# 2361098148/LocoManipulationRL

Hardware: AMD Instinct MI355X
Metric: env-steps/sec (whole node), horizontal-locomotion 4096 envs (higher is better)
Workload: dtype f32

## Files before the change

locomanipulationrl_amd/csrc/lm_dynamics.h:

```cpp
#pragma once
#include "lm_samplers.h"

#if defined(LM_STAMPS) && LM_STAMPS != 2
#define LM_STAMP(k) do { __builtin_amdgcn_sched_barrier(0); unsigned long long t_; \
    asm volatile("s_memtime %0\n\ts_waitcnt lgkmcnt(0)" : "=s"(t_) :: "memory"); __builtin_amdgcn_sched_barrier(0); \
    if (threadIdx.x == 0) { lm_stamp_lds[k] += t_ - lm_stamp_lds[15]; lm_stamp_lds[15] = t_; } } while (0)
#else
#define LM_STAMP(k) do { } while (0)
#endif

#define HUB_FLOATS 10
#define ENVS_PER_WAVE 16
#define PUB_LIMB_STRIDE 123
#define LIMB_STRIDE 124
#define T_J0 0
#define T_P1 14
#define T_P2 40
#define T_I0 66
#define T_Q1 76
#define T_Q2 96
#define T_TIP 116
#define T_FOOT 119
#define T_FLAG 122
#define LM_ITAB_FLOATS (HUB_FLOATS + 4 * LIMB_STRIDE)
// ... 243 lines not shown
    Wf[0] = Wl[0] + b0; Wf[1] = Wl[1] + a0.x; Wf[2] = Wl[2] + a0.y;
    Wf[3] = Wl[3] + a1.x; Wf[4] = Wl[4] + a1.y; Wf[5] = Wl[5] + a2.y;
  }
  const float imu = mu > 0.f ? 1.0f / mu : 0.f;
  const float nrW0 = -1.0f / Wf[0]; G.W0t = mk2(Wf[1], Wf[2]); G.nrWt = mk2(-imu / Wf[3], -imu / Wf[5]);
  pgs_cross_blocks<0>(limb, T, X, Wf, G.X0[0], G.X12[0]); pgs_cross_blocks<1>(limb, T, X, Wf, G.X0[1], G.X12[1]);
  pgs_cross_blocks<2>(limb, T, X, Wf, G.X0[2], G.X12[2]); pgs_cross_blocks<3>(limb, T, X, Wf, G.X0[3], G.X12[3]);
#pragma unroll
  for (int k = 0; k < 4; k++) { G.X0[k][0] *= nrW0; G.X0[k][1] *= mu * nrW0; G.X0[k][2] *= mu * nrW0; G.X12[k][1] = sp2(mu) * G.X12[k][1]; G.X12[k][2] = sp2(mu) * G.X12[k][2]; }
  S.lam0 = 0.f; S.lam12 = sp2(0.f);
  S.c0 = (vf[0] + bn) * nrW0; S.c12 = mk2(vf[1], vf[2]);
  S.m0 = limb == 0 ? 1.f : 0.f; S.m1 = limb == 1 ? 1.f : 0.f; S.m2 = limb == 2 ? 1.f : 0.f; S.m3 = limb == 3 ? 1.f : 0.f;
}
LM_DEV void pgs_sweeps(PgsState& S, int it0, int it1) {
  for (int it = it0; it < it1; it += 2) {
    pgs_turn<0>(S.m0, S.G, S.lam0, S.lam12, S.c0, S.c12);
    pgs_turn<1>(S.m1, S.G, S.lam0, S.lam12, S.c0, S.c12);
    pgs_turn<2>(S.m2, S.G, S.lam0, S.lam12, S.c0, S.c12);
    pgs_turn<3>(S.m3, S.G, S.lam0, S.lam12, S.c0, S.c12);
    if (it + 1 < it1) {
      pgs_turn<3>(S.m3, S.G, S.lam0, S.lam12, S.c0, S.c12);
      pgs_turn<2>(S.m2, S.G, S.lam0, S.lam12, S.c0, S.c12);
      pgs_turn<1>(S.m1, S.G, S.lam0, S.lam12, S.c0, S.c12);
      pgs_turn<0>(S.m0, S.G, S.lam0, S.lam12, S.c0, S.c12);
    }
  }
}
LM_DEV void pgs_finish(const PgsState& S, float mu, const R4 X[6], float lam[3], float w[6]) {
  const f2 l12 = sp2(mu) * S.lam12;
  lam[0] = S.lam0; lam[1] = l12.x; lam[2] = l12.y;
#pragma unroll
  for (int i = 0; i < 6; i++) { const f2 t = l12 * X[i].q; w[i] = quad_sum(fmaf(S.lam0, X[i].p.y, t.x + t.y)); }
}

struct FreeBody { V3 p; Q4 q; SV u; };

LM_DEV void integrate_free(FreeBody& F, const M3& R, float dt) {
  V3 ww = mul(R, F.u.w);
  float wn = sqrtf(dot(ww, ww)), th = wn * dt;
  Q4 dq;
  if (th < 1e-8f) { dq.w = 1.f; dq.x = 0.5f * dt * ww.x; dq.y = 0.5f * dt * ww.y; dq.z = 0.5f * dt * ww.z; }
  else { float sh, ch; lm_sincos(0.5f * th, &sh, &ch); float s = sh / wn; dq.w = ch; dq.x = s * ww.x; dq.y = s * ww.y; dq.z = s * ww.z; }
  Q4 qn = qmul(dq, F.q);
  float rn = rsqrtf(qn.w * qn.w + qn.x * qn.x + qn.y * qn.y + qn.z * qn.z);
  F.q.w = qn.w * rn; F.q.x = qn.x * rn; F.q.y = qn.y * rn; F.q.z = qn.z * rn;
  M3 Rn = quat_to_mat(F.q.w, F.q.x, F.q.y, F.q.z);
  F.p = fma3(dt, mul(Rn, F.u.v), F.p);
}

#ifdef LM_WAVES2
#define STASH_SLOTS 18
#define LM_STEP_ATTR __attribute__((amdgpu_waves_per_eu(2, 2)))
#elif defined(LM_HELPER_WAVE)
#define STASH_SLOTS 29
#define HAND_IN 22
#define HAND_OUT 26
#define LM_STEP_ATTR
#else
#define STASH_SLOTS 22
#define LM_STEP_ATTR
#endif
struct Stash {
  float4* base; int lane;
  LM_DEV void put(int slot, float a, float b, float c, float d) const { base[slot * 64 + lane] = make_float4(a, b, c, d); }
  LM_DEV float4 get(int slot) const { return base[slot * 64 + lane]; }
};
#ifdef LM_HELPER_WAVE
LM_DEV void hw_barrier() {
  __builtin_amdgcn_sched_barrier(0);
  asm volatile("" ::: "memory");
  __builtin_amdgcn_s_waitcnt(0xc07f);
  __builtin_amdgcn_s_barrier();
  asm volatile("" ::: "memory");
  __builtin_amdgcn_sched_barrier(0);
}
#endif
LM_DEV void stash_sv3(const Stash& S, int slot, SV a, SV b, SV c, float e0 = 0.f, float e1 = 0.f) {
  S.put(slot + 0, a.w.x, a.w.y, a.w.z, a.v.x); S.put(slot + 1, a.v.y, a.v.z, b.w.x, b.w.y);
  S.put(slot + 2, b.w.z, b.v.x, b.v.y, b.v.z); S.put(slot + 3, c.w.x, c.w.y, c.w.z, c.v.x); S.put(slot + 4, c.v.y, c.v.z, e0, e1);
}
LM_DEV void unstash_sv3(const Stash& S, int slot, SV& a, SV& b, SV& c) {
  float4 t0 = S.get(slot), t1 = S.get(slot + 1), t2 = S.get(slot + 2), t3 = S.get(slot + 3), t4 = S.get(slot + 4);
  a = sv(v3(t0.x, t0.y, t0.z), v3(t0.w, t1.x, t1.y)); b = sv(v3(t1.z, t1.w, t2.x), v3(t2.y, t2.z, t2.w)); c = sv(v3(t3.x, t3.y, t3.z), v3(t3.w, t4.x, t4.y));
}

#if defined(LM_PASS0_STASH) || defined(LM_WAVES2)
#define LM_PASS0_REG 0
#else
#define LM_PASS0_REG 1
#endif
struct PassTerms {
  S6 Fq0, Fq1, Fq2;
  float Ha[6], hq[3];
  float Jq0[3]; f2 j12[3];
  R4 PB[6];
  SI Isc;
};
LM_DEV S6 s6(SV a) { S6 r; r.a = mk2(a.w.x, a.w.y); r.b = mk2(a.w.z, a.v.x); r.c = mk2(a.v.y, a.v.z); return r; }
#define LM_PASS_ROWS(I, b, r0, r1, r2) { \
  I.PB[0].p = mk2(b.w.x, r0.w.x); I.PB[1].p = mk2(b.w.y, r0.w.y); I.PB[2].p = mk2(b.w.z, r0.w.z); \
  I.PB[3].p = mk2(b.v.x, r0.v.x); I.PB[4].p = mk2(b.v.y, r0.v.y); I.PB[5].p = mk2(b.v.z, r0.v.z); \
  I.PB[0].q = mk2(r1.w.x, r2.w.x); I.PB[1].q = mk2(r1.w.y, r2.w.y); I.PB[2].q = mk2(r1.w.z, r2.w.z); \
  I.PB[3].q = mk2(r1.v.x, r2.v.x); I.PB[4].q = mk2(r1.v.y, r2.v.y); I.PB[5].q = mk2(r1.v.z, r2.v.z); }
LM_DEV void pin(float& x) { asm("" : "+v"(x)); }
LM_DEV void pin(f2& x) { asm("" : "+v"(x)); }
LM_DEV void pin(S6& x) { pin(x.a); pin(x.b); pin(x.c); }
template <int MODE> LM_DEV void pin_terms(PassTerms& I) {
  pin(I.Fq0); pin(I.Fq1); pin(I.Fq2);
  pin(I.Ha[0]); pin(I.Ha[1]); pin(I.Ha[2]); pin(I.Ha[3]); pin(I.Ha[4]); pin(I.Ha[5]);
  pin(I.hq[0]); pin(I.hq[1]); pin(I.hq[2]); pin(I.Jq0[0]); pin(I.Jq0[1]); pin(I.Jq0[2]); pin(I.j12[0]); pin(I.j12[1]); pin(I.j12[2]);
  pin(I.PB[0].p); pin(I.PB[1].p); pin(I.PB[2].p); pin(I.PB[3].p); pin(I.PB[4].p); pin(I.PB[5].p);
  pin(I.PB[0].q); pin(I.PB[1].q); pin(I.PB[2].q); pin(I.PB[3].q); pin(I.PB[4].q); pin(I.PB[5].q);
  if (MODE == 0) { pin(I.Isc.m); pin(I.Isc.h.x); pin(I.Isc.h.y); pin(I.Isc.h.z); pin(I.Isc.xx); pin(I.Isc.yy); pin(I.Isc.zz); pin(I.Isc.xy); pin(I.Isc.xz); pin(I.Isc.yz); }
// ... 29 lines not shown
  St.put(4, I.Fq2.c.x, I.Fq2.c.y, 0.f, 0.f);
  St.put(5, I.Ha[0], I.Ha[1], I.Ha[2], I.Ha[3]); St.put(6, I.Ha[4], I.Ha[5], 0.f, 0.f);
  St.put(16, I.Isc.m, I.Isc.h.x, I.Isc.h.y, I.Isc.h.z); St.put(17, I.Isc.xx, I.Isc.yy, I.Isc.zz, I.Isc.xy); St.put(18, I.Isc.xz, I.Isc.yz, 0.f, 0.f);
}
#endif
template <int MODE> LM_DEV void unstash_terms(const Stash& St, PassTerms& I) {
  asm volatile("" ::: "memory");
  float isc_xz = 0.f, isc_yz = 0.f;
  {
    const float4 t0 = St.get(0), t1 = St.get(1), t2 = St.get(2), t3 = St.get(3), t4 = St.get(4);
    isc_xz = t4.z; isc_yz = t4.w;
    I.Fq0.a = mk2(t0.x, t0.y); I.Fq0.b = mk2(t0.z, t0.w); I.Fq0.c = mk2(t1.x, t1.y);
    I.Fq1.a = mk2(t1.z, t1.w); I.Fq1.b = mk2(t2.x, t2.y); I.Fq1.c = mk2(t2.z, t2.w);
    I.Fq2.a = mk2(t3.x, t3.y); I.Fq2.b = mk2(t3.z, t3.w); I.Fq2.c = mk2(t4.x, t4.y);
  }
  const float4 h5 = St.get(5), h6 = St.get(6), h7 = St.get(7), h8 = St.get(8), h9 = St.get(9);
  I.Ha[0] = h5.x; I.Ha[1] = h5.y; I.Ha[2] = h5.z; I.Ha[3] = h5.w; I.Ha[4] = h6.x; I.Ha[5] = h6.y;
  I.hq[0] = h6.z; I.hq[1] = h6.w; I.hq[2] = h7.x;
  I.Jq0[0] = h7.y; I.Jq0[1] = h7.z; I.Jq0[2] = h7.w;
  I.j12[0] = mk2(h8.x, h8.y); I.j12[1] = mk2(h8.z, h8.w); I.j12[2] = mk2(h9.x, h9.y);
  {
    const float4 g0 = St.get(10), g1 = St.get(11), g2 = St.get(12), g3 = St.get(13), g4 = St.get(14), g5 = St.get(15);
    I.PB[0].p = mk2(g0.x, g0.y); I.PB[1].p = mk2(g0.z, g0.w); I.PB[2].p = mk2(g1.x, g1.y); I.PB[3].p = mk2(g1.z, g1.w); I.PB[4].p = mk2(g2.x, g2.y); I.PB[5].p = mk2(g2.z, g2.w);
    I.PB[0].q = mk2(g3.x, g3.y); I.PB[1].q = mk2(g3.z, g3.w); I.PB[2].q = mk2(g4.x, g4.y); I.PB[3].q = mk2(g4.z, g4.w); I.PB[4].q = mk2(g5.x, g5.y); I.PB[5].q = mk2(g5.z, g5.w);
  }
  if (MODE == 0) {
#ifdef LM_WAVES2
    const float4 g16 = St.get(16), g17 = St.get(17), g18 = make_float4(isc_xz, isc_yz, 0.f, 0.f);
#else
    const float4 g16 = St.get(16), g17 = St.get(17), g18 = St.get(18); (void)isc_xz; (void)isc_yz;
#endif
    I.Isc.m = g16.x; I.Isc.h = v3(g16.y, g16.z, g16.w); I.Isc.xx = g17.x; I.Isc.yy = g17.y; I.Isc.zz = g17.z; I.Isc.xy = g17.w; I.Isc.xz = g18.x; I.Isc.yz = g18.y;
  }
}

template <class T> struct PlateInvT { V3T<T> ii, c; T im; };
LM_DEV PlateInvT<float> plate_inv(const lm_params* __restrict__ P, float m, float s) {
  PlateInvT<float> Q; Q.ii = v3(1.0f / (s * P->plate_inertia[0]), 1.0f / (s * P->plate_inertia[1]), 1.0f / (s * P->plate_inertia[2]));
  Q.c = v3(P->plate_com[0], P->plate_com[1], P->plate_com[2]); Q.im = 1.0f / m; return Q;
}
template <class T> LM_DEV void plate_inv_apply(const PlateInvT<T>& Q, V3T<T> n, V3T<T> f, V3T<T>& al, V3T<T>& a) {
  const V3T<T> nc = n - cross(Q.c, f);
  al = v3t<T>(nc.x * Q.ii.x, nc.y * Q.ii.y, nc.z * Q.ii.z);
  a = fma3(Q.im, f, cross(Q.c, al));
}
LM_DEV SI plate_inertia_env(const lm_params* __restrict__ P, float m, float s) {
  const V3 c = v3(P->plate_com[0], P->plate_com[1], P->plate_com[2]); const float cc = dot(c, c);
  SI I; I.m = m; I.h = m * c;
  I.xx = fmaf(m, cc - c.x * c.x, s * P->plate_inertia[0]); I.yy = fmaf(m, cc - c.y * c.y, s * P->plate_inertia[1]); I.zz = fmaf(m, cc - c.z * c.z, s * P->plate_inertia[2]);
  I.xy = -m * c.x * c.y; I.xz = -m * c.x * c.z; I.yz = -m * c.y * c.z;
  return I;
}

template <int MODE, int VAR, int DR, int CF, int HW = 0>
LM_DEV void substep_pass(const lm_params* __restrict__ P, int limb, const FreeBody& F, const PassTerms& I, float dt, float kd, const float cjv[3],
                         const bool sat[3], const float tsat[3], const float tgt[3], const float qd[3], float bn, float mu_dr,
                         bool mp_on, float m_plate, float s_plate, float qdn[3], SV& un, float lamc[3], const Stash* Hd = nullptr) {
  const S6 Fq0 = I.Fq0, Fq1 = I.Fq1, Fq2 = I.Fq2;
  float Ha[6] = {I.Ha[0], I.Ha[1], I.Ha[2], I.Ha[3], I.Ha[4], I.Ha[5]}, r[3];
  const float hq[3] = {I.hq[0], I.hq[1], I.hq[2]};
  R4 PBh[6];
  const float Jq_[3][3] = {{I.Jq0[0], I.Jq0[1], I.Jq0[2]}, {I.j12[0].x, I.j12[1].x, I.j12[2].x}, {I.j12[0].y, I.j12[1].y, I.j12[2].y}};
  const f2 j12_[3] = {I.j12[0], I.j12[1], I.j12[2]};
  float Jqh[3][3]; f2 j12h[3]; float bnh = bn;
  const float (*Jq)[3] = HW == 2 ? Jqh : Jq_;
  const f2* j12 = HW == 2 ? j12h : j12_;
  const R4* PB = HW ? PBh : I.PB;
  const int di[3] = {0, 3, 5};
#pragma unroll
  for (int a = 0; a < 3; a++) {
    const float cj = cjv[a];
    {
#pragma clang fp contract(off)
      Ha[di[a]] = fmaf(dt, sat[a] ? cj : kd + cj, Ha[di[a]]);
      const float rr = sat[a] ? tsat[a] : kd * (tgt[a] - qd[a]);
      const float damp = cj * qd[a];
      r[a] = HW ? rr - damp : (rr - damp) - hq[a];
    }
  }
  float Hi[6]; inv3sym(Ha, Hi);
  const S6 K0 = fma6(Hi[0], Fq0, fma6(Hi[1], Fq1, Hi[2] * Fq2));
  const S6 K1 = fma6(Hi[1], Fq0, fma6(Hi[3], Fq1, Hi[4] * Fq2));
  const S6 K2 = fma6(Hi[2], Fq0, fma6(Hi[4], Fq1, Hi[5] * Fq2));
  float qdd[3], qdf[3], v0f[6], vf[3];
  R4 T[6], X[6];
  if (MODE == 0) {
    float A0[6][6]; si_to_66(I.Isc, A0);
    float A[6][6];
#define LM_AROW(I) { \
      const f2 k0 = sp2(comp<I>(K0)), k1 = sp2(comp<I>(K1)), k2 = sp2(comp<I>(K2)); \
      _Pragma("unroll") for (int jp = (I) / 2; jp < 3; jp++) { \
        const f2 f0 = jp == 0 ? Fq0.a : jp == 1 ? Fq0.b : Fq0.c, f1 = jp == 0 ? Fq1.a : jp == 1 ? Fq1.b : Fq1.c, f2_ = jp == 0 ? Fq2.a : jp == 1 ? Fq2.b : Fq2.c; \
        const f2 v = fma_(-k2, f2_, fma_(-k1, f1, fma_(-k0, f0, mk2(A0[I][2 * jp], A0[I][2 * jp + 1])))); \
        if (2 * jp >= (I)) A[I][2 * jp] = quad_sum(v.x); \
        A[I][2 * jp + 1] = quad_sum(v.y); } }
    LM_AROW(0) LM_AROW(1) LM_AROW(2) LM_AROW(3) LM_AROW(4) LM_AROW(5)
#undef LM_AROW
#ifdef LM_HELPER_WAVE
    if (HW) {
      hw_barrier();
      const float4 b0 = Hd->get(HAND_OUT), b1 = Hd->get(HAND_OUT + 1), b2 = Hd->get(HAND_OUT + 2);
      const float fcs[6] = {b0.x, b0.y, b0.z, b0.w, b1.x, b1.y}, hqh[3] = {b1.z, b1.w, b2.x};
      if (HW == 2) {
        const float4 t7 = Hd->get(7), t8 = Hd->get(8), t9 = Hd->get(9);
        const float4 g0 = Hd->get(10), g1 = Hd->get(11), g2 = Hd->get(12), g3 = Hd->get(13), g4 = Hd->get(14), g5 = Hd->get(15);
        j12h[0] = mk2(t8.x, t8.y); j12h[1] = mk2(t8.z, t8.w); j12h[2] = mk2(t9.x, t9.y); bnh = t9.z;
        Jqh[0][0] = t7.y; Jqh[0][1] = t7.z; Jqh[0][2] = t7.w;
#pragma unroll
        for (int c = 0; c < 3; c++) { Jqh[1][c] = j12h[c].x; Jqh[2][c] = j12h[c].y; }
        PBh[0].p = mk2(fcs[0], g0.y); PBh[1].p = mk2(fcs[1], g0.w); PBh[2].p = mk2(fcs[2], g1.y);
        PBh[3].p = mk2(fcs[3], g1.w); PBh[4].p = mk2(fcs[4], g2.y); PBh[5].p = mk2(fcs[5], g2.w);
        PBh[0].q = mk2(g3.x, g3.y); PBh[1].q = mk2(g3.z, g3.w); PBh[2].q = mk2(g4.x, g4.y);
        PBh[3].q = mk2(g4.z, g4.w); PBh[4].q = mk2(g5.x, g5.y); PBh[5].q = mk2(g5.z, g5.w);
      } else {
#pragma unroll
      for (int i = 0; i < 6; i++) { PBh[i].p = mk2(fcs[i], I.PB[i].p.y); PBh[i].q = I.PB[i].q; }
      }
#pragma unroll
      for (int a = 0; a < 3; a++) {
#pragma clang fp contract(off)
        r[a] = r[a] - hqh[a];
      }
    }
#endif
    Chol6 Ch; chol6(A, Ch);
    const f2 cp[3] = {mk2(r[0], -Jq[0][0]), mk2(r[1], -Jq[0][1]), mk2(r[2], -Jq[0][2])};
#define LM_PROW(I) { \
      const f2 k0 = sp2(comp<I>(K0)), k1 = sp2(comp<I>(K1)), k2 = sp2(comp<I>(K2)); \
      T[I].p = fma_(cp[2], k2, fma_(cp[1], k1, fma_(cp[0], k0, PB[I].p))); \
      T[I].q = fma_(-j12[2], k2, fma_(-j12[1], k1, fma_(-j12[0], k0, PB[I].q))); \
      X[I].p = mk2(-quad_sum(T[I].p.x), T[I].p.y); X[I].q = T[I].q; }
    LM_PROW(0) LM_PROW(1) LM_PROW(2) LM_PROW(3) LM_PROW(4) LM_PROW(5)
#undef LM_PROW
    chol6_solve4(Ch, X);
    float t0 = r[0], t1 = r[1], t2 = r[2];
#define LM_TROW(I) { const float a = X[I].p.x; t0 = fmaf(-comp<I>(Fq0), a, t0); t1 = fmaf(-comp<I>(Fq1), a, t1); t2 = fmaf(-comp<I>(Fq2), a, t2); }
    LM_TROW(0) LM_TROW(1) LM_TROW(2) LM_TROW(3) LM_TROW(4) LM_TROW(5)
#undef LM_TROW
    qdd[0] = Hi[0] * t0 + Hi[1] * t1 + Hi[2] * t2; qdd[1] = Hi[1] * t0 + Hi[3] * t1 + Hi[4] * t2; qdd[2] = Hi[2] * t0 + Hi[4] * t1 + Hi[5] * t2;
    const float u6[6] = {F.u.w.x, F.u.w.y, F.u.w.z, F.u.v.x, F.u.v.y, F.u.v.z};
#pragma unroll
    for (int i = 0; i < 6; i++) v0f[i] = fmaf(dt, X[i].p.x, u6[i]);
  } else {
    qdd[0] = Hi[0] * r[0] + Hi[1] * r[1] + Hi[2] * r[2]; qdd[1] = Hi[1] * r[0] + Hi[3] * r[1] + Hi[4] * r[2]; qdd[2] = Hi[2] * r[0] + Hi[4] * r[1] + Hi[5] * r[2];
#pragma unroll
    for (int i = 0; i < 6; i++) { v0f[i] = PB[i].p.x; T[i] = PB[i]; }
    if (mp_on) {
      const PlateInvT<float> Q1 = plate_inv(P, m_plate, s_plate);
      PlateInvT<f2> Q; Q.ii = bc(Q1.ii); Q.c = bc(Q1.c); Q.im = sp2(Q1.im);
      V3P al, ac;
      plate_inv_apply<f2>(Q, v3(T[0].p, T[1].p, T[2].p), v3(T[3].p, T[4].p, T[5].p), al, ac);
      X[0].p = al.x; X[1].p = al.y; X[2].p = al.z; X[3].p = ac.x; X[4].p = ac.y; X[5].p = ac.z;
      plate_inv_apply<f2>(Q, v3(T[0].q, T[1].q, T[2].q), v3(T[3].q, T[4].q, T[5].q), al, ac);
      X[0].q = al.x; X[1].q = al.y; X[2].q = al.z; X[3].q = ac.x; X[4].q = ac.y; X[5].q = ac.z;
    } else {
#pragma unroll
    for (int i = 0; i < 6; i++) {
      f2 bp = sp2(0.f), bq = sp2(0.f);
#pragma unroll
      for (int j = 0; j < 6; j++) { const f2 ph = sp2(P->plate_phi[6 * i + j]); bp = fma_(ph, T[j].p, bp); bq = fma_(ph, T[j].q, bq); }
      X[i].p = bp; X[i].q = bq;
    }
    }
  }
#pragma unroll
  for (int a = 0; a < 3; a++) qdf[a] = fmaf(dt, qdd[a], qd[a]);
  float Wl[6];
  float JH[3][3];
#pragma unroll
  for (int rr = 0; rr < 3; rr++) {
    JH[rr][0] = Jq[rr][0] * Hi[0] + Jq[rr][1] * Hi[1] + Jq[rr][2] * Hi[2];
    JH[rr][1] = Jq[rr][0] * Hi[1] + Jq[rr][1] * Hi[3] + Jq[rr][2] * Hi[4];
    JH[rr][2] = Jq[rr][0] * Hi[2] + Jq[rr][1] * Hi[4] + Jq[rr][2] * Hi[5];
  }
  Wl[0] = JH[0][0] * Jq[0][0] + JH[0][1] * Jq[0][1] + JH[0][2] * Jq[0][2];
  Wl[1] = JH[0][0] * Jq[1][0] + JH[0][1] * Jq[1][1] + JH[0][2] * Jq[1][2];
  Wl[2] = JH[0][0] * Jq[2][0] + JH[0][1] * Jq[2][1] + JH[0][2] * Jq[2][2];
  Wl[3] = JH[1][0] * Jq[1][0] + JH[1][1] * Jq[1][1] + JH[1][2] * Jq[1][2];
  Wl[4] = JH[1][0] * Jq[2][0] + JH[1][1] * Jq[2][1] + JH[1][2] * Jq[2][2];
  Wl[5] = JH[2][0] * Jq[2][0] + JH[2][1] * Jq[2][1] + JH[2][2] * Jq[2][2];
  {
    float a = 0.f; f2 b = sp2(0.f);
#pragma unroll
    for (int i = 0; i < 6; i++) { a = fmaf(PB[i].p.y, v0f[i], a); b = fma_(PB[i].q, sp2(v0f[i]), b); }
    vf[0] = a + (Jq[0][0] * qdf[0] + Jq[0][1] * qdf[1] + Jq[0][2] * qdf[2]);
    vf[1] = b.x + (Jq[1][0] * qdf[0] + Jq[1][1] * qdf[1] + Jq[1][2] * qdf[2]);
    vf[2] = b.y + (Jq[2][0] * qdf[0] + Jq[2][1] * qdf[1] + Jq[2][2] * qdf[2]);
  }
  float lam[3], w[6];
  LM_STAMP(3);
  PgsState S; pgs_setup(S, limb, DR ? mu_dr : P->mu, HW == 2 ? bnh : bn, vf, Wl, T, X);
  pgs_sweeps(S, 0, P->pgs_iters);
  pgs_finish(S, DR ? mu_dr : P->mu, X, lam, w);
  if (CF) { lamc[0] = lam[0]; lamc[1] = lam[1]; lamc[2] = lam[2]; }
  un = sv(v3(v0f[0] + w[0], v0f[1] + w[1], v0f[2] + w[2]), v3(v0f[3] + w[3], v0f[4] + w[4], v0f[5] + w[5]));
#pragma unroll
  for (int a = 0; a < 3; a++) qdn[a] = qdf[a] + JH[0][a] * lam[0] + JH[1][a] * lam[1] + JH[2][a] * lam[2];
  if (MODE == 0) {
#define LM_WROW(I) { qdn[0] = fmaf(-comp<I>(K0), w[I], qdn[0]); qdn[1] = fmaf(-comp<I>(K1), w[I], qdn[1]); qdn[2] = fmaf(-comp<I>(K2), w[I], qdn[2]); }
    LM_WROW(0) LM_WROW(1) LM_WROW(2) LM_WROW(3) LM_WROW(4) LM_WROW(5)
#undef LM_WROW
  }
  LM_STAMP(4);
}

#ifdef LM_HELPER_WAVE
LM_DEV void helper_wave(const lm_params* __restrict__ P, const float* sTab, float4* sStash, int lane, int nsub) {
  const int limb = lane & 3;
  const float* th = sTab; const float* tl = sTab + HUB_FLOATS + limb * LIMB_STRIDE;
  Stash St; St.base = sStash; St.lane = lane;
  const float gravity = P->gravity;
  for (int s = 0; s < nsub; s++) {
    hw_barrier();
    const float4 h0 = St.get(HAND_IN), h1 = St.get(HAND_IN + 1), h2 = St.get(HAND_IN + 2), h3 = St.get(HAND_IN + 3);
    const float q[3] = {h0.x, h0.y, h0.z}, qd[3] = {h0.w, h1.x, h1.y};
    const SV v0 = sv(v3(h1.z, h1.w, h2.x), v3(h2.y, h2.z, h2.w));
    const SV avp0 = sv(v3(0, 0, 0), gravity * v3(h3.x, h3.y, h3.z));
    LimbKin K; limb_kinematics(tl, q, qd, K);
    LimbDyn D; limb_dynamics<0, 2>(tl, K, qd, v0, avp0, D);
    {
      const float m0 = (limb == 0) ? 1.f : 0.f;
      SI I0 = hub_inertia(th);
      I0.m *= m0; I0.h = m0 * I0.h; I0.xx *= m0; I0.yy *= m0; I0.zz *= m0; I0.xy *= m0; I0.xz *= m0; I0.yz *= m0;
      D.fcs = D.fcs + I0 * avp0 + fcross(v0, I0 * v0);
    }
    St.put(HAND_OUT, D.fcs.w.x, D.fcs.w.y, D.fcs.w.z, D.fcs.v.x); St.put(HAND_OUT + 1, D.fcs.v.y, D.fcs.v.z, D.hq[0], D.hq[1]); St.put(HAND_OUT + 2, D.hq[2], 0.f, 0.f, 0.f);
    hw_barrier();
  }
}
#if LM_HELPER_WAVE >= 2
LM_DEV void helper_wave_terms(const lm_params* __restrict__ P, const float* sTab, float4* sStash, int lane, int nsub) {
  const int limb = lane & 3;
  const float* tl = sTab + HUB_FLOATS + limb * LIMB_STRIDE;
  Stash St; St.base = sStash; St.lane = lane;
  const float dt = P->dt, baumgarte = P->baumgarte, max_depen_vel = P->max_depen_vel;
  for (int s = 0; s < nsub; s++) {
    hw_barrier();
    const float4 h0 = St.get(HAND_IN), h1 = St.get(HAND_IN + 1), h2 = St.get(HAND_IN + 2), h3 = St.get(HAND_IN + 3);
    const float q[3] = {h0.x, h0.y, h0.z}, qd[3] = {h0.w, h1.x, h1.y};
    const SV v0 = sv(v3(h1.z, h1.w, h2.x), v3(h2.y, h2.z, h2.w));
    const SV avp0 = sv(v3(0, 0, 0), v3(0, 0, 0));
    LimbKin K; limb_kinematics(tl, q, qd, K);
    LimbDyn D; limb_dynamics<0, 1>(tl, K, qd, v0, avp0, D);
    V3 C0, C1, C2; float phi;
    C0 = v3(h3.x, h3.y, h3.z);
    C1 = rsqrtf(fmaxf(1.0f - C0.x * C0.x, 1.0e-12f)) * v3(1.0f - C0.x * C0.x, -C0.x * C0.y, -C0.x * C0.z);
    C2 = cross(C0, C1);
    phi = h3.w + dot(C0, D.x) - P->tip_radius;
    D.x = fma3(-P->tip_radius, C0, D.x);
    const float bn = (phi >= 0.f) ? phi / dt : fmaxf(baumgarte * phi / dt, -max_depen_vel);
    V3 e0 = K.s1.v + cross(K.s1.w, D.x);
    V3 e1 = D.j31.v + cross(D.j31.w, D.x);
    V3 e2 = D.j32.v + cross(D.j32.w, D.x);
    St.put(7, 0.f, dot(C0, e0), dot(C0, e1), dot(C0, e2));
    St.put(8, dot(C1, e0), dot(C2, e0), dot(C1, e1), dot(C2, e1)); St.put(9, dot(C1, e2), dot(C2, e2), bn, 0.f);
    const V3 n0 = cross(D.x, C0), n1 = cross(D.x, C1), n2 = cross(D.x, C2);
    St.put(10, 0.f, n0.x, 0.f, n0.y); St.put(11, 0.f, n0.z, 0.f, C0.x); St.put(12, 0.f, C0.y, 0.f, C0.z);
    St.put(13, n1.x, n2.x, n1.y, n2.y); St.put(14, n1.z, n2.z, C1.x, C2.x); St.put(15, C1.y, C2.y, C1.z, C2.z);
    hw_barrier();
  }
}
#endif
#endif

template <int MODE, int VAR, int DR, int CF = 0, int REG0 = 1, int HW = 0>
LM_DEV void substep(const lm_params* __restrict__ P, const float* th, const float* tl, int limb, const Stash& St,
                    FreeBody& F, const M3& Rfix, V3 pfix, float q[3], float qd[3], const float tgt[3], float tau_acc[3], const DrPhys& X, float* cf = nullptr) {
  const float dt = P->dt, kd = DR ? X.kd : P->kd;
  const float cjv[3] = {VAR ? (DR ? X.cj[0] : P->joint_damping) : 0.f, VAR ? (DR ? X.cj[1] : P->joint_damping) : 0.f, VAR ? (DR ? X.cj[2] : P->joint_damping) : 0.f};
  const float tmax[3] = {DR ? X.tmax[0] : P->tau_max, DR ? X.tmax[1] : P->tau_max, DR ? X.tmax[2] : P->tau_max};
  const float mu_dr = DR ? X.mu : 0.f;
  const bool mp_on = DR && MODE == 1 && X.mp_on;
  const float m_plate = mp_on ? X.m_plate : 0.f, s_plate = mp_on ? X.s_plate : 0.f;
  M3 Rf = quat_to_mat(F.q.w, F.q.x, F.q.y, F.q.z);
#ifdef LM_HELPER_WAVE
  static_assert(!HW || (MODE == 0 && !DR && LM_PASS0_REG && REG0), "the helper wavefront serves the un-randomised locomotion sub-step with its first pass on registers");
  if (HW) {
    St.put(HAND_IN, q[0], q[1], q[2], qd[0]); St.put(HAND_IN + 1, qd[1], qd[2], F.u.w.x, F.u.w.y); St.put(HAND_IN + 2, F.u.w.z, F.u.v.x, F.u.v.y, F.u.v.z);
    St.put(HAND_IN + 3, Rf.c0.z, Rf.c1.z, Rf.c2.z, HW == 2 ? F.p.z : 0.f);
    hw_barrier();
  }
#endif
  constexpr bool REG0_ = LM_PASS0_REG ? REG0 != 0 : false;
  const float baumgarte = REG0_ ? P->baumgarte : 0.f, max_depen_vel = REG0_ ? P->max_depen_vel : 0.f;
  float bn; PassTerms I;
  {
    M3 Rb; V3 pb; SV v0;
    if (MODE == 0) { Rb = Rf; pb = F.p; v0 = F.u; } else { Rb = Rfix; pb = pfix; v0 = sv(v3(0, 0, 0), v3(0, 0, 0)); }
    SV avp0 = sv(v3(0, 0, 0), DR ? mulT(Rb, -X.g) : P->gravity * row2(Rb));
    LimbKin K; limb_kinematics(tl, q, qd, K);
    LimbDyn D;
    if (DR && X.mb_on) limb_dynamics<1>(tl, K, qd, v0, avp0, D, X.m_s, X.m_41, X.m_32);
    else if (HW) limb_dynamics<0, 1>(tl, K, qd, v0, avp0, D);
    else limb_dynamics(tl, K, qd, v0, avp0, D);
    LM_STAMP(1);
    if (MODE == 0) {
      const float m0 = (limb == 0) ? 1.f : 0.f;
      SI I0 = hub_inertia(th);
      if (DR && X.mb_on) {
        const V3 c = (1.0f / I0.m) * I0.h; const float dm = X.m_hub - I0.m, cc = dot(c, c);
        I0.xx = fmaf(dm, cc - c.x * c.x, I0.xx); I0.yy = fmaf(dm, cc - c.y * c.y, I0.yy); I0.zz = fmaf(dm, cc - c.z * c.z, I0.zz);
        I0.xy = fmaf(dm, -(c.x * c.y), I0.xy); I0.xz = fmaf(dm, -(c.x * c.z), I0.xz); I0.yz = fmaf(dm, -(c.y * c.z), I0.yz);
        I0.h = (X.m_hub / I0.m) * I0.h; I0.m = X.m_hub;
      }
      const V3 com0 = (1.0f / I0.m) * I0.h;
      I0.m *= m0; I0.h = m0 * I0.h; I0.xx *= m0; I0.yy *= m0; I0.zz *= m0; I0.xy *= m0; I0.xz *= m0; I0.yz *= m0;
      D.Isc = D.Isc + I0;
      if (!HW) D.fcs = D.fcs + I0 * avp0 + fcross(v0, I0 * v0);
      if (DR) { V3 fh = m0 * mulT(Rb, X.f); D.fcs = D.fcs - sv(cross(com0, fh), fh); }
    }
#ifdef LM_HELPER_WAVE
    if (HW == 2) {
      I.Fq0 = s6(D.Fq0); I.Fq1 = s6(D.Fq1); I.Fq2 = s6(D.Fq2);
      I.Ha[0] = D.H[0]; I.Ha[1] = D.H[1]; I.Ha[2] = D.H[2]; I.Ha[3] = D.H[3]; I.Ha[4] = D.H[4]; I.Ha[5] = D.H[5];
      I.hq[0] = I.hq[1] = I.hq[2] = 0.f; I.Jq0[0] = I.Jq0[1] = I.Jq0[2] = 0.f; I.j12[0] = I.j12[1] = I.j12[2] = sp2(0.f);
#pragma unroll
      for (int i = 0; i < 6; i++) { I.PB[i].p = sp2(0.f); I.PB[i].q = sp2(0.f); }
      I.Isc = D.Isc;
      pin_chain(I);
      stash_chain(St, I);
      bn = 0.f;
    }
#endif
    if (HW != 2) {
    V3 C0, C1, C2;
    float phi;
    if (MODE == 0) {
      C0 = row2(Rb);
      C1 = rsqrtf(fmaxf(1.0f - C0.x * C0.x, 1.0e-12f)) * v3(1.0f - C0.x * C0.x, -C0.x * C0.y, -C0.x * C0.z);
      C2 = cross(C0, C1);
      phi = pb.z + dot(C0, D.x) - P->tip_radius;
      D.x = fma3(-P->tip_radius, C0, D.x);
    } else {
      V3 xw = pb + mul(Rb, D.x);
      V3 yc = mulT(Rf, xw - F.p);
      V3 y = yc - v3(P->plate_center[0], P->plate_center[1], P->plate_center[2]);
      float sg = (mulT(Rf, pb - F.p).z - P->plate_center[2] >= 0.f) ? 1.f : -1.f;
      phi = sg * y.z - P->plate_half[2] - P->tip_radius;
      if (fabsf(y.x) > P->plate_half[0] || fabsf(y.y) > P->plate_half[1]) phi = 1.0e3f;
      M3 Mrp = mulTA(Rb, Rf);
      C0 = sg * Mrp.c2; C1 = Mrp.c0; C2 = sg * Mrp.c1;
      D.x = fma3(-P->tip_radius, C0, D.x);
      V3 y0 = v3(yc.x, yc.y, yc.z - sg * P->tip_radius);
      V3 a0 = v3(0, 0, sg), a1 = v3(1, 0, 0), a2 = v3(0, sg, 0);
      SV Tp0 = sv(-cross(y0, a0), -a0), Tp1 = sv(-cross(y0, a1), -a1), Tp2 = sv(-cross(y0, a2), -a2);
      SV up_free;
      if (mp_on) {
        const V3 c = v3(P->plate_com[0], P->plate_com[1], P->plate_com[2]);
        const SI Ip = plate_inertia_env(P, m_plate, s_plate);
        SV hp = fcross(F.u, Ip * F.u);
        const V3 fg = m_plate * mulT(Rf, X.g);
        hp = hp - sv(cross(c, fg), fg);
        const PlateInvT<float> Q = plate_inv(P, m_plate, s_plate);
        V3 al, ac; plate_inv_apply<float>(Q, hp.w, hp.v, al, ac);
        up_free = F.u - dt * sv(al, ac);
      } else {
        SI Ip = load_si(P->plate_si);
        SV hp = fcross(F.u, Ip * F.u);
        V3 fg = DR ? P->plate_mass * mulT(Rf, X.g) : (-P->plate_mass * P->gravity) * row2(Rf);
        V3 c = v3(P->plate_com[0], P->plate_com[1], P->plate_com[2]);
        hp = hp - sv(cross(c, fg), fg);
        float Ph[6][6];
#pragma unroll
        for (int i = 0; i < 6; i++)
#pragma unroll
          for (int j = 0; j < 6; j++) Ph[i][j] = P->plate_phi[6 * i + j];
        up_free = F.u - dt * mul66(Ph, hp);
      }
      if (!REG0_) {
        St.put(10, up_free.w.x, Tp0.w.x, up_free.w.y, Tp0.w.y); St.put(11, up_free.w.z, Tp0.w.z, up_free.v.x, Tp0.v.x); St.put(12, up_free.v.y, Tp0.v.y, up_free.v.z, Tp0.v.z);
        St.put(13, Tp1.w.x, Tp2.w.x, Tp1.w.y, Tp2.w.y); St.put(14, Tp1.w.z, Tp2.w.z, Tp1.v.x, Tp2.v.x); St.put(15, Tp1.v.y, Tp2.v.y, Tp1.v.z, Tp2.v.z);
      } else LM_PASS_ROWS(I, up_free, Tp0, Tp1, Tp2)
    }
    bn = (phi >= 0.f) ? phi / dt : REG0_ ? fmaxf(baumgarte * phi / dt, -max_depen_vel) : fmaxf(P->baumgarte * phi / dt, -P->max_depen_vel);
    V3 e0 = K.s1.v + cross(K.s1.w, D.x);
    V3 e1 = D.j31.v + cross(D.j31.w, D.x);
    V3 e2 = D.j32.v + cross(D.j32.w, D.x);
// ... 34 lines not shown
      pin_terms<MODE>(I);
      stash_terms<MODE>(St, I);
    }
    }
  }

  LM_STAMP(2);
  const bool effort = (VAR == 0) && P->drive_mode == LM_DRIVE_EFFORT;
  bool sat[3] = {effort, effort, effort}; float tsat[3] = {effort ? tgt[0] : 0.f, effort ? tgt[1] : 0.f, effort ? tgt[2] : 0.f};
  if (VAR) {
#pragma unroll
    for (int a = 0; a < 3; a++) {
      const float tau = kd * (tgt[a] - qd[a]);
      const bool hi_ = tau > tmax[a], lo_ = tau < -tmax[a];
      sat[a] = hi_ || lo_; tsat[a] = hi_ ? tmax[a] : -tmax[a];
    }
  }
  float qdn[3]; SV un; float lamc[3] = {0.f, 0.f, 0.f};
  auto second_pass_due = [&]() -> bool {
    if (effort || (VAR != 0 && !P->pd_second_pass)) return false;
    int any = 0;
#pragma unroll
    for (int a = 0; a < 3; a++) {
      const float tau = kd * (tgt[a] - qdn[a]);
      const bool hi_ = tau > tmax[a], lo_ = tau < -tmax[a];
      if (VAR) {
        const bool nw = !sat[a] && (hi_ || lo_);
        tsat[a] = nw ? (hi_ ? tmax[a] : -tmax[a]) : tsat[a]; sat[a] = sat[a] || nw; any |= nw ? 1 : 0;
      } else {
        sat[a] = hi_ || lo_; tsat[a] = hi_ ? tmax[a] : -tmax[a]; any |= (hi_ || lo_) ? 1 : 0;
      }
    }
    any = quad_sum_i(any);
#ifdef LM_COUNT_PASS2
    { const bool wa = __any(any); if ((threadIdx.x & 63) == 0) { atomicAdd(&lm_dbg_pass2[0], 1u); if (wa) atomicAdd(&lm_dbg_pass2[1], 1u); } }
#endif
    return __any(any);
  };
  if (!REG0_) {
    for (int pass = 0; pass < 2; pass++) {
      unstash_terms<MODE>(St, I);
      substep_pass<MODE, VAR, DR, CF>(P, limb, F, I, dt, kd, cjv, sat, tsat, tgt, qd, bn, mu_dr, mp_on, m_plate, s_plate, qdn, un, lamc);
      if (pass == 0 && !second_pass_due()) break;
    }
  } else {
    substep_pass<MODE, VAR, DR, CF, HW>(P, limb, F, I, dt, kd, cjv, sat, tsat, tgt, qd, bn, mu_dr, mp_on, m_plate, s_plate, qdn, un, lamc, &St);
    if (second_pass_due()) {
      unstash_terms<MODE>(St, I);
#ifdef LM_HELPER_WAVE
      if (HW) {
        const float4 b0 = St.get(HAND_OUT), b1 = St.get(HAND_OUT + 1), b2 = St.get(HAND_OUT + 2);
        I.PB[0].p.x = b0.x; I.PB[1].p.x = b0.y; I.PB[2].p.x = b0.z; I.PB[3].p.x = b0.w; I.PB[4].p.x = b1.x; I.PB[5].p.x = b1.y;
        I.hq[0] = b1.z; I.hq[1] = b1.w; I.hq[2] = b2.x;
        if (HW == 2) bn = St.get(9).z;
      }
#endif
      substep_pass<MODE, VAR, DR, CF>(P, limb, F, I, dt, kd, cjv, sat, tsat, tgt, qd, bn, mu_dr, mp_on, m_plate, s_plate, qdn, un, lamc);
    }
  }
#pragma unroll
  for (int a = 0; a < 3; a++) {
    if (VAR) tau_acc[a] += sat[a] ? tsat[a] : fminf(fmaxf(kd * (tgt[a] - qdn[a]), -tmax[a]), tmax[a]);
    const float vm = DR ? X.vmax[a] : P->max_joint_vel;
    float v = fminf(fmaxf(qdn[a], -vm), vm);
    qd[a] = v; q[a] = fmaf(dt, v, q[a]);
  }
  if (CF) {
    if (MODE == 0) {
      const float s = rsqrtf(fmaxf(fmaf(-Rf.c0.z, Rf.c0.z, 1.0f), 1.0e-12f));
      cf[0] = fmaf(s, fmaf(lamc[1], Rf.c0.x, -(lamc[2] * Rf.c0.y)), cf[0]);
      cf[1] = fmaf(s, fmaf(lamc[1], Rf.c0.y, lamc[2] * Rf.c0.x), cf[1]);
      cf[2] += lamc[0];
    } else {
      const float sg = (mulT(Rf, pfix - F.p).z - P->plate_center[2] >= 0.f) ? 1.f : -1.f;
      const float ln = sg * lamc[0], l2 = sg * lamc[2];
      cf[0] += fmaf(ln, Rf.c2.x, fmaf(lamc[1], Rf.c0.x, l2 * Rf.c1.x));
      cf[1] += fmaf(ln, Rf.c2.y, fmaf(lamc[1], Rf.c0.y, l2 * Rf.c1.y));
      cf[2] += fmaf(ln, Rf.c2.z, fmaf(lamc[1], Rf.c0.z, l2 * Rf.c1.z));
    }
    cf[3] += lamc[0] > 0.f ? 1.f : 0.f;
  }
  F.u = un;
  integrate_free(F, Rf, dt);
  LM_STAMP(5);
}

LM_DEV void store_contact(float* rec, int N, int env, int limb, bool active, const float cf[4], int n, float dt) {
  if (!active || n <= 0) return;
  const float sc = 1.0f / ((float)n * dt);
  rec[(size_t)(3 * limb + 0) * N + env] = cf[0] * sc; rec[(size_t)(3 * limb + 1) * N + env] = cf[1] * sc; rec[(size_t)(3 * limb + 2) * N + env] = cf[2] * sc;
  rec[(size_t)(12 + limb) * N + env] = (float)((double)cf[3] / (double)n);
}
```

locomanipulationrl_amd/csrc/lm_engine_h3.hip:

```cpp
#ifndef LM_HELPER_WAVE
#define LM_HELPER_WAVE 2
#endif
#ifndef LM_H3_OUT_HELPER
#define LM_H3_OUT_HELPER 1
#endif
#undef LM_STAMPS
#undef LM_COUNT_PASS2
#undef LM_WAVES2
#undef LM_PASS0_STASH
#include "lm_step.h"

__global__ void __launch_bounds__(192) k_step_h3(StepArgs A) {
  LM_STEP_SMEM(64)
  if (threadIdx.x >= 64) {
    const int nsub = (A.nsub < 0) ? P->substeps : A.nsub;
    if (kind != 0 || env0 >= A.N) return;
    if (threadIdx.x >= 128) {
      helper_wave_terms(P, sTab, sStash, threadIdx.x - 128, nsub);
      if (LM_H3_OUT_HELPER) helper_write_outputs<64>(P, A.W, A.N, env0, threadIdx.x - 128, sObs, sSt);
    } else helper_wave(P, sTab, sStash, threadIdx.x - 64, nsub);
    return;
  }
  if (kind == 0) step_body<0, 0, 0, 0, 0, 1, 2, LM_H3_OUT_HELPER>(A, P, sTab, sObs, sSt, sStash); else step_body<1, 0, 0>(A, P, sTab, sObs, sSt, sStash);
}
extern "C" __attribute__((visibility("hidden"))) void lm_internal_launch_step_h3(const StepArgs* A, int nblocks, hipStream_t s) {
  hipLaunchKernelGGL(k_step_h3, dim3(nblocks), dim3(192), 0, s, *A);
}
```

Before: 146.4 million.

## Add fourth helper wavefront computing hub Schur complement and Cholesky factor

Adds a fourth wavefront per block (256 threads) that recomputes the limb kinematics and dynamics from the handed-in joint state. It then forms the 6x6 hub Schur complement, factors it with Cholesky, and passes the factor through LDS stash slots. The main wavefront skips building and factoring that matrix and only reads the result after a barrier. This moves work off the critical path, at the cost of extra LDS stash space, more threads per block, duplicated kinematics work and an extra barrier participant, which may reduce occupancy.

```diff
diff --git a/locomanipulationrl_amd/csrc/lm_dynamics.h b/locomanipulationrl_amd/csrc/lm_dynamics.h
--- a/locomanipulationrl_amd/csrc/lm_dynamics.h
+++ b/locomanipulationrl_amd/csrc/lm_dynamics.h
@@ -319,13 +319,21 @@
 #define STASH_SLOTS 18
 #define LM_STEP_ATTR __attribute__((amdgpu_waves_per_eu(2, 2)))
 #elif defined(LM_HELPER_WAVE)
+#if LM_HELPER_WAVE >= 3
+#define STASH_SLOTS 35
+#else
 #define STASH_SLOTS 29
+#endif
 #define HAND_IN 22
 #define HAND_OUT 26
+#define HAND_HUB 29
 #define LM_STEP_ATTR
 #else
 #define STASH_SLOTS 22
 #define LM_STEP_ATTR
+#endif
+#ifndef LM_H3_HUB_CHOL
+#define LM_H3_HUB_CHOL 1
 #endif
 struct Stash {
   float4* base; int lane;
@@ -461,6 +469,25 @@
   return I;
 }
 
+
+#define LM_AROW(I) { \
+      const f2 k0 = sp2(comp<I>(K0)), k1 = sp2(comp<I>(K1)), k2 = sp2(comp<I>(K2)); \
+      _Pragma("unroll") for (int jp = (I) / 2; jp < 3; jp++) { \
+        const f2 f0 = jp == 0 ? Fq0.a : jp == 1 ? Fq0.b : Fq0.c, f1 = jp == 0 ? Fq1.a : jp == 1 ? Fq1.b : Fq1.c, f2_ = jp == 0 ? Fq2.a : jp == 1 ? Fq2.b : Fq2.c; \
+        const f2 v = fma_(-k2, f2_, fma_(-k1, f1, fma_(-k0, f0, mk2(A0[I][2 * jp], A0[I][2 * jp + 1])))); \
+        if (2 * jp >= (I)) A[I][2 * jp] = quad_sum(v.x); \
+        A[I][2 * jp + 1] = quad_sum(v.y); } }
+#ifdef LM_HELPER_WAVE
+LM_DEV void hub_put(const Stash& St, const float* h) {
+  St.put(HAND_HUB, h[0], h[1], h[2], h[3]); St.put(HAND_HUB + 1, h[4], h[5], h[6], h[7]); St.put(HAND_HUB + 2, h[8], h[9], h[10], h[11]);
+  St.put(HAND_HUB + 3, h[12], h[13], h[14], h[15]); St.put(HAND_HUB + 4, h[16], h[17], h[18], h[19]); St.put(HAND_HUB + 5, h[20], 0.f, 0.f, 0.f);
+}
+LM_DEV void hub_get(const Stash& St, float* h) {
+  const float4 c0 = St.get(HAND_HUB), c1 = St.get(HAND_HUB + 1), c2 = St.get(HAND_HUB + 2), c3 = St.get(HAND_HUB + 3), c4 = St.get(HAND_HUB + 4), c5 = St.get(HAND_HUB + 5);
+  h[0] = c0.x; h[1] = c0.y; h[2] = c0.z; h[3] = c0.w; h[4] = c1.x; h[5] = c1.y; h[6] = c1.z; h[7] = c1.w; h[8] = c2.x; h[9] = c2.y; h[10] = c2.z; h[11] = c2.w;
+  h[12] = c3.x; h[13] = c3.y; h[14] = c3.z; h[15] = c3.w; h[16] = c4.x; h[17] = c4.y; h[18] = c4.z; h[19] = c4.w; h[20] = c5.x;
+}
+#endif
 template <int MODE, int VAR, int DR, int CF, int HW = 0>
 LM_DEV void substep_pass(const lm_params* __restrict__ P, int limb, const FreeBody& F, const PassTerms& I, float dt, float kd, const float cjv[3],
                          const bool sat[3], const float tsat[3], const float tgt[3], const float qd[3], float bn, float mu_dr,
@@ -472,8 +499,8 @@
   const float Jq_[3][3] = {{I.Jq0[0], I.Jq0[1], I.Jq0[2]}, {I.j12[0].x, I.j12[1].x, I.j12[2].x}, {I.j12[0].y, I.j12[1].y, I.j12[2].y}};
   const f2 j12_[3] = {I.j12[0], I.j12[1], I.j12[2]};
   float Jqh[3][3]; f2 j12h[3]; float bnh = bn;
-  const float (*Jq)[3] = HW == 2 ? Jqh : Jq_;
-  const f2* j12 = HW == 2 ? j12h : j12_;
+  const float (*Jq)[3] = HW >= 2 ? Jqh : Jq_;
+  const f2* j12 = HW >= 2 ? j12h : j12_;
   const R4* PB = HW ? PBh : I.PB;
   const int di[3] = {0, 3, 5};
 #pragma unroll
@@ -488,29 +515,41 @@
     }
   }
   float Hi[6]; inv3sym(Ha, Hi);
-  const S6 K0 = fma6(Hi[0], Fq0, fma6(Hi[1], Fq1, Hi[2] * Fq2));
-  const S6 K1 = fma6(Hi[1], Fq0, fma6(Hi[3], Fq1, Hi[4] * Fq2));
-  const S6 K2 = fma6(Hi[2], Fq0, fma6(Hi[4], Fq1, Hi[5] * Fq2));
+  S6 K0 = fma6(Hi[0], Fq0, fma6(Hi[1], Fq1, Hi[2] * Fq2));
+  S6 K1 = fma6(Hi[1], Fq0, fma6(Hi[3], Fq1, Hi[4] * Fq2));
+  S6 K2 = fma6(Hi[2], Fq0, fma6(Hi[4], Fq1, Hi[5] * Fq2));
   float qdd[3], qdf[3], v0f[6], vf[3];
   R4 T[6], X[6];
   if (MODE == 0) {
-    float A0[6][6]; si_to_66(I.Isc, A0);
-    float A[6][6];
-#define LM_AROW(I) { \
-      const f2 k0 = sp2(comp<I>(K0)), k1 = sp2(comp<I>(K1)), k2 = sp2(comp<I>(K2)); \
-      _Pragma("unroll") for (int jp = (I) / 2; jp < 3; jp++) { \
-        const f2 f0 = jp == 0 ? Fq0.a : jp == 1 ? Fq0.b : Fq0.c, f1 = jp == 0 ? Fq1.a : jp == 1 ? Fq1.b : Fq1.c, f2_ = jp == 0 ? Fq2.a : jp == 1 ? Fq2.b : Fq2.c; \
-        const f2 v = fma_(-k2, f2_, fma_(-k1, f1, fma_(-k0, f0, mk2(A0[I][2 * jp], A0[I][2 * jp + 1])))); \
-        if (2 * jp >= (I)) A[I][2 * jp] = quad_sum(v.x); \
-        A[I][2 * jp + 1] = quad_sum(v.y); } }
-    LM_AROW(0) LM_AROW(1) LM_AROW(2) LM_AROW(3) LM_AROW(4) LM_AROW(5)
-#undef LM_AROW
+    float A[6][6]; Chol6 Ch;
+    if (HW < 3) {
+      float A0[6][6]; si_to_66(I.Isc, A0);
+      LM_AROW(0) LM_AROW(1) LM_AROW(2) LM_AROW(3) LM_AROW(4) LM_AROW(5)
+    }
 #ifdef LM_HELPER_WAVE
     if (HW) {
+      if (HW == 3) { pin(K0); pin(K1); pin(K2); }
       hw_barrier();
       const float4 b0 = Hd->get(HAND_OUT), b1 = Hd->get(HAND_OUT + 1), b2 = Hd->get(HAND_OUT + 2);
       const float fcs[6] = {b0.x, b0.y, b0.z, b0.w, b1.x, b1.y}, hqh[3] = {b1.z, b1.w, b2.x};
-      if (HW == 2) {
+      if (HW == 3) {
+        float h[21]; hub_get(*Hd, h);
+        int n = 0;
+        if (LM_H3_HUB_CHOL) {
+#pragma unroll
+          for (int i = 1; i < 6; i++)
+#pragma unroll
+            for (int k = 0; k < i; k++) Ch.L[i][k] = h[n++];
+#pragma unroll
+          for (int i = 0; i < 6; i++) Ch.d[i] = h[n++];
+        } else {
+#pragma unroll
+          for (int i = 0; i < 6; i++)
+#pragma unroll
+            for (int j = i; j < 6; j++) A[i][j] = h[n++];
+        }
+      }
+      if (HW >= 2) {
         const float4 t7 = Hd->get(7), t8 = Hd->get(8), t9 = Hd->get(9);
         const float4 g0 = Hd->get(10), g1 = Hd->get(11), g2 = Hd->get(12), g3 = Hd->get(13), g4 = Hd->get(14), g5 = Hd->get(15);
         j12h[0] = mk2(t8.x, t8.y); j12h[1] = mk2(t8.z, t8.w); j12h[2] = mk2(t9.x, t9.y); bnh = t9.z;
@@ -532,7 +571,7 @@
       }
     }
 #endif
-    Chol6 Ch; chol6(A, Ch);
+    if (!(HW == 3 && LM_H3_HUB_CHOL)) chol6(A, Ch);
     const f2 cp[3] = {mk2(r[0], -Jq[0][0]), mk2(r[1], -Jq[0][1]), mk2(r[2], -Jq[0][2])};
 #define LM_PROW(I) { \
       const f2 k0 = sp2(comp<I>(K0)), k1 = sp2(comp<I>(K1)), k2 = sp2(comp<I>(K2)); \
@@ -598,7 +637,7 @@
   }
   float lam[3], w[6];
   LM_STAMP(3);
-  PgsState S; pgs_setup(S, limb, DR ? mu_dr : P->mu, HW == 2 ? bnh : bn, vf, Wl, T, X);
+  PgsState S; pgs_setup(S, limb, DR ? mu_dr : P->mu, HW >= 2 ? bnh : bn, vf, Wl, T, X);
   pgs_sweeps(S, 0, P->pgs_iters);
   pgs_finish(S, DR ? mu_dr : P->mu, X, lam, w);
   if (CF) { lamc[0] = lam[0]; lamc[1] = lam[1]; lamc[2] = lam[2]; }
@@ -670,7 +709,72 @@
   }
 }
 #endif
-#endif
+#if LM_HELPER_WAVE >= 3
+LM_DEV void helper_wave_hub(const lm_params* __restrict__ P, const float* sTab, float4* sStash, int lane, int nsub) {
+  const int limb = lane & 3;
+  const float* th = sTab; const float* tl = sTab + HUB_FLOATS + limb * LIMB_STRIDE;
+  Stash St; St.base = sStash; St.lane = lane;
+  const float dt = P->dt, kd = P->kd;
+  const bool effort = P->drive_mode == LM_DRIVE_EFFORT;
+  for (int s = 0; s < nsub; s++) {
+    hw_barrier();
+    const float4 h0 = St.get(HAND_IN), h1 = St.get(HAND_IN + 1);
+    const float q[3] = {h0.x, h0.y, h0.z}, qd[3] = {h0.w, h1.x, h1.y};
+    const SV v0 = sv(v3(0, 0, 0), v3(0, 0, 0)), avp0 = v0;
+    LimbKin K; limb_kinematics(tl, q, qd, K);
+    LimbDyn D; limb_dynamics<0, 1>(tl, K, qd, v0, avp0, D);
+    {
+      const float m0 = (limb == 0) ? 1.f : 0.f;
+      SI I0 = hub_inertia(th);
+      I0.m *= m0; I0.h = m0 * I0.h; I0.xx *= m0; I0.yy *= m0; I0.zz *= m0; I0.xy *= m0; I0.xz *= m0; I0.yz *= m0;
+      D.Isc = D.Isc + I0;
+    }
+    PassTerms I;
+    I.Fq0 = s6(D.Fq0); I.Fq1 = s6(D.Fq1); I.Fq2 = s6(D.Fq2);
+    I.Ha[0] = D.H[0]; I.Ha[1] = D.H[1]; I.Ha[2] = D.H[2]; I.Ha[3] = D.H[3]; I.Ha[4] = D.H[4]; I.Ha[5] = D.H[5];
+    I.Isc = D.Isc;
+    pin_chain(I);
+    const S6 Fq0 = I.Fq0, Fq1 = I.Fq1, Fq2 = I.Fq2;
+    float Ha[6] = {I.Ha[0], I.Ha[1], I.Ha[2], I.Ha[3], I.Ha[4], I.Ha[5]};
+    const bool sat[3] = {effort, effort, effort};
+    const int di[3] = {0, 3, 5};
+#pragma unroll
+    for (int a = 0; a < 3; a++) {
+      const float cj = 0.f;
+      {
+#pragma clang fp contract(off)
+        Ha[di[a]] = fmaf(dt, sat[a] ? cj : kd + cj, Ha[di[a]]);
+      }
+    }
+    float Hi[6]; inv3sym(Ha, Hi);
+    const S6 K0 = fma6(Hi[0], Fq0, fma6(Hi[1], Fq1, Hi[2] * Fq2));
+    const S6 K1 = fma6(Hi[1], Fq0, fma6(Hi[3], Fq1, Hi[4] * Fq2));
+    const S6 K2 = fma6(Hi[2], Fq0, fma6(Hi[4], Fq1, Hi[5] * Fq2));
+    float A0[6][6]; si_to_66(I.Isc, A0);
+    float A[6][6];
+    LM_AROW(0) LM_AROW(1) LM_AROW(2) LM_AROW(3) LM_AROW(4) LM_AROW(5)
+    float h[21]; int n = 0;
+    if (LM_H3_HUB_CHOL) {
+      Chol6 Ch; chol6(A, Ch);
+#pragma unroll
+      for (int i = 1; i < 6; i++)
+#pragma unroll
+        for (int k = 0; k < i; k++) h[n++] = Ch.L[i][k];
+#pragma unroll
+      for (int i = 0; i < 6; i++) h[n++] = Ch.d[i];
+    } else {
+#pragma unroll
+      for (int i = 0; i < 6; i++)
+#pragma unroll
+        for (int j = i; j < 6; j++) h[n++] = A[i][j];
+    }
+    hub_put(St, h);
+    hw_barrier();
+  }
+}
+#endif
+#endif
+#undef LM_AROW
 
 template <int MODE, int VAR, int DR, int CF = 0, int REG0 = 1, int HW = 0>
 LM_DEV void substep(const lm_params* __restrict__ P, const float* th, const float* tl, int limb, const Stash& St,
@@ -686,7 +790,7 @@
   static_assert(!HW || (MODE == 0 && !DR && LM_PASS0_REG && REG0), "the helper wavefront serves the un-randomised locomotion sub-step with its first pass on registers");
   if (HW) {
     St.put(HAND_IN, q[0], q[1], q[2], qd[0]); St.put(HAND_IN + 1, qd[1], qd[2], F.u.w.x, F.u.w.y); St.put(HAND_IN + 2, F.u.w.z, F.u.v.x, F.u.v.y, F.u.v.z);
-    St.put(HAND_IN + 3, Rf.c0.z, Rf.c1.z, Rf.c2.z, HW == 2 ? F.p.z : 0.f);
+    St.put(HAND_IN + 3, Rf.c0.z, Rf.c1.z, Rf.c2.z, HW >= 2 ? F.p.z : 0.f);
     hw_barrier();
   }
 #endif
@@ -719,7 +823,7 @@
       if (DR) { V3 fh = m0 * mulT(Rb, X.f); D.fcs = D.fcs - sv(cross(com0, fh), fh); }
     }
 #ifdef LM_HELPER_WAVE
-    if (HW == 2) {
+    if (HW >= 2) {
       I.Fq0 = s6(D.Fq0); I.Fq1 = s6(D.Fq1); I.Fq2 = s6(D.Fq2);
       I.Ha[0] = D.H[0]; I.Ha[1] = D.H[1]; I.Ha[2] = D.H[2]; I.Ha[3] = D.H[3]; I.Ha[4] = D.H[4]; I.Ha[5] = D.H[5];
       I.hq[0] = I.hq[1] = I.hq[2] = 0.f; I.Jq0[0] = I.Jq0[1] = I.Jq0[2] = 0.f; I.j12[0] = I.j12[1] = I.j12[2] = sp2(0.f);
@@ -731,7 +835,7 @@
       bn = 0.f;
     }
 #endif
-    if (HW != 2) {
+    if (HW < 2) {
     V3 C0, C1, C2;
     float phi;
     if (MODE == 0) {
@@ -872,7 +976,7 @@
         const float4 b0 = St.get(HAND_OUT), b1 = St.get(HAND_OUT + 1), b2 = St.get(HAND_OUT + 2);
         I.PB[0].p.x = b0.x; I.PB[1].p.x = b0.y; I.PB[2].p.x = b0.z; I.PB[3].p.x = b0.w; I.PB[4].p.x = b1.x; I.PB[5].p.x = b1.y;
         I.hq[0] = b1.z; I.hq[1] = b1.w; I.hq[2] = b2.x;
-        if (HW == 2) bn = St.get(9).z;
+        if (HW >= 2) bn = St.get(9).z;
       }
 #endif
       substep_pass<MODE, VAR, DR, CF>(P, limb, F, I, dt, kd, cjv, sat, tsat, tgt, qd, bn, mu_dr, mp_on, m_plate, s_plate, qdn, un, lamc);
diff --git a/locomanipulationrl_amd/csrc/lm_engine_h3.hip b/locomanipulationrl_amd/csrc/lm_engine_h3.hip
--- a/locomanipulationrl_amd/csrc/lm_engine_h3.hip
+++ b/locomanipulationrl_amd/csrc/lm_engine_h3.hip
@@ -1,5 +1,12 @@
+#ifndef LM_H3_HUB_HELPER
+#define LM_H3_HUB_HELPER 1
+#endif
 #ifndef LM_HELPER_WAVE
+#if LM_H3_HUB_HELPER
+#define LM_HELPER_WAVE 3
+#else
 #define LM_HELPER_WAVE 2
+#endif
 #endif
 #ifndef LM_H3_OUT_HELPER
 #define LM_H3_OUT_HELPER 1
@@ -10,19 +17,24 @@
 #undef LM_PASS0_STASH
 #include "lm_step.h"
 
-__global__ void __launch_bounds__(192) k_step_h3(StepArgs A) {
+#define LM_H3_THREADS (LM_H3_HUB_HELPER ? 256 : 192)
+
+__global__ void __launch_bounds__(LM_H3_THREADS) k_step_h3(StepArgs A) {
   LM_STEP_SMEM(64)
   if (threadIdx.x >= 64) {
     const int nsub = (A.nsub < 0) ? P->substeps : A.nsub;
     if (kind != 0 || env0 >= A.N) return;
+#if LM_H3_HUB_HELPER
+    if (threadIdx.x >= 192) { helper_wave_hub(P, sTab, sStash, threadIdx.x - 192, nsub); return; }
+#endif
     if (threadIdx.x >= 128) {
       helper_wave_terms(P, sTab, sStash, threadIdx.x - 128, nsub);
       if (LM_H3_OUT_HELPER) helper_write_outputs<64>(P, A.W, A.N, env0, threadIdx.x - 128, sObs, sSt);
     } else helper_wave(P, sTab, sStash, threadIdx.x - 64, nsub);
     return;
   }
-  if (kind == 0) step_body<0, 0, 0, 0, 0, 1, 2, LM_H3_OUT_HELPER>(A, P, sTab, sObs, sSt, sStash); else step_body<1, 0, 0>(A, P, sTab, sObs, sSt, sStash);
+  if (kind == 0) step_body<0, 0, 0, 0, 0, 1, LM_HELPER_WAVE, LM_H3_OUT_HELPER>(A, P, sTab, sObs, sSt, sStash); else step_body<1, 0, 0>(A, P, sTab, sObs, sSt, sStash);
 }
 extern "C" __attribute__((visibility("hidden"))) void lm_internal_launch_step_h3(const StepArgs* A, int nblocks, hipStream_t s) {
-  hipLaunchKernelGGL(k_step_h3, dim3(nblocks), dim3(192), 0, s, *A);
+  hipLaunchKernelGGL(k_step_h3, dim3(nblocks), dim3(LM_H3_THREADS), 0, s, *A);
 }
```

Result: no change. 147.1 million, median of 6 (+0.5%).
